# PalamaraLab/FastSMC

Measured on AMD Instinct MI355X. Metric: haplotype-pairs decoded/sec (whole node) + GB/s vs HBM roofline, 69-state HMM, higher is better.
Workload: dtype f32; 1 GPU; synthetic 1000 haplotypes x 50000 sites, K=69, all 499500 pairs per GPU, FastSMC-mode IBD + posterior-mean/MAP ages, no hashing; mode=ibd, resident_waves=2048, n_cu=256, chunk_sites=512, chunks_per_window=98, resident_chunks=24, beta_stride=2, kernel_member=69, record_gather=none, lib_hash=414cfd5268fcdcb0

## Files before the change

### fastsmc_amd/capi.py

```python
from __future__ import annotations

import ctypes as C
import operator
import os

import numpy as np

_HERE = os.path.dirname(os.path.abspath(__file__))
LIB_PATH = os.environ.get("FSMC_HIP_LIB") or os.path.join(_HERE, "libfastsmc_hip.so")

FSMC_WANT_MEAN = 1
FSMC_WANT_MAP = 2
FSMC_WANT_SUMS = 4
FSMC_WANT_MAJOR_MINOR_SUMS = 8

FSMC_EOVERFLOW = -6

SYMBOLS = [
    "fsmc_ctx_create", "fsmc_ctx_destroy", "fsmc_last_error", "fsmc_ctx_info", "fsmc_ctx_set_workspace_limit",
    "fsmc_ctx_expect_work",
    "fsmc_ctx_set_chunk_sites", "fsmc_ctx_set_beta_stride", "fsmc_ctx_last_beta_stride", "fsmc_ctx_last_plan",
    "fsmc_ctx_last_kernel", "fsmc_ctx_set_pairing", "fsmc_ctx_last_items", "fsmc_ctx_set_two_wave_windows", "fsmc_ctx_last_waves_per_window", "fsmc_ctx_last_segment_sums_in_lds", "fsmc_ctx_set_resident_chunks",
    "fsmc_ctx_last_resident_chunks", "fsmc_ctx_set_chunk_pool", "fsmc_ctx_last_chunk_pool",
    "fsmc_model_create", "fsmc_model_destroy", "fsmc_haps_upload", "fsmc_worklist_upload",
    "fsmc_decode_ibd_launch", "fsmc_decode_ibd_fetch", "fsmc_sync", "fsmc_last_kernel_ms", "fsmc_phase_cycles",
    "fsmc_decode_ibd",
    "fsmc_decode_posteriors", "fsmc_decode_per_pair", "fsmc_decode_sums", "fsmc_decode_sums_batches",
    "fsmc_decode_pair_posteriors", "fsmc_ctx_set_pair_posterior_slice", "fsmc_ctx_last_pair_posterior_slices",
    "fsmc_decode_pair_minima", "fsmc_ctx_set_pair_minima_slice", "fsmc_ctx_last_pair_minima_slices",
    "fsmc_decode_pair_bins", "fsmc_ctx_set_pair_bins_slice", "fsmc_ctx_last_pair_bins_slices",
    "fsmc_decode_pair_cdf", "fsmc_ctx_set_pair_cdf_slice", "fsmc_ctx_last_pair_cdf_slices",
    "fsmc_decode_pair_tail_summaries", "fsmc_ctx_set_pair_tail_slice", "fsmc_ctx_last_pair_tail_slices",
    "fsmc_decode_pair_loglik", "fsmc_ctx_set_pair_loglik_slice", "fsmc_ctx_last_pair_loglik_slices",
    "fsmc_decode_pair_viterbi", "fsmc_ctx_set_pair_viterbi_slice", "fsmc_ctx_last_pair_viterbi_slices",
    "fsmc_decode_pair_samples", "fsmc_ctx_set_pair_samples_slice", "fsmc_ctx_last_pair_samples_slices",
    "fsmc_identify", "fsmc_identify_ex", "fsmc_identify_fetch",
]

PAIR_DTYPE = np.dtype([("hap_a", "<u4"), ("hap_b", "<u4")])
GROUP_DTYPE = np.dtype([("first_pair", "<u4"), ("n_pairs", "<u4"), ("from", "<u4"), ("to", "<u4"),
                        ("scan_from", "<u4"), ("scan_to", "<u4")])
CANDIDATE_DTYPE = np.dtype([("hap_a", "<u4"), ("hap_b", "<u4"), ("from", "<u4"), ("to", "<u4"), ("flush_word", "<u4")])
IBD_DTYPE = np.dtype([("pair", "<u4"), ("start", "<i4"), ("end", "<i4"), ("prob", "<f4"), ("post_mean", "<f4"),
                      ("map", "<f4")])


def log_likelihood(mant, expo):
    with np.errstate(divide="ignore"):
        return np.log(np.asarray(mant, np.float64)) + np.asarray(expo, np.float64) * np.log(2.0)


class FsmcError(RuntimeError):
    def __init__(self, code: int, msg: str):
# ... 13 lines not shown

class _ModelDesc(C.Structure):
    _fields_ = [
        ("K", C.c_int32), ("S", C.c_int32),
        ("pi", C.c_void_p), ("col_ratios", C.c_void_p), ("exp_times", C.c_void_p),
        ("n_rows", C.c_int32),
        ("D", C.c_void_p), ("B", C.c_void_p), ("U", C.c_void_p), ("RR", C.c_void_p),
        ("step_row", C.c_void_p),
        ("e1", C.c_void_p), ("e0m1", C.c_void_p), ("e2m0", C.c_void_p),
        ("state_threshold", C.c_uint32), ("age_threshold", C.c_uint32), ("probability_threshold", C.c_float),
        ("sequence", C.c_int32),
        ("gap_row_f", C.c_void_p), ("site_row_f", C.c_void_p), ("gap_row_b", C.c_void_p), ("site_row_b", C.c_void_p),
        ("hom", C.c_void_p),
    ]


_lib = None


def load():
    global _lib
    if _lib is None:
        if not os.path.exists(LIB_PATH):
            raise FsmcError(-100, f"{LIB_PATH} is missing: build it with `python -c 'import __graft_entry__ as g; "
                                  "g.build()'` (there is no CPU fallback)")
        L = C.CDLL(LIB_PATH)
        vp, i32, u32, u64, sz = C.c_void_p, C.c_int32, C.c_uint32, C.c_uint64, C.c_size_t
        L.fsmc_ctx_create.argtypes = [C.c_int, vp, C.POINTER(vp)]
        L.fsmc_ctx_destroy.argtypes = [vp]
        L.fsmc_ctx_destroy.restype = None
        L.fsmc_last_error.argtypes = [vp]
        L.fsmc_last_error.restype = C.c_char_p
        L.fsmc_ctx_info.argtypes = [vp, C.POINTER(i32), C.POINTER(i32), C.POINTER(u64)]
        L.fsmc_ctx_set_workspace_limit.argtypes = [vp, u64]
        L.fsmc_ctx_expect_work.argtypes = [vp, C.c_double, C.c_int32]
        L.fsmc_ctx_set_chunk_sites.argtypes = [vp, u32]
        L.fsmc_ctx_set_beta_stride.argtypes = [vp, u32]
        L.fsmc_ctx_last_beta_stride.argtypes = [vp, C.POINTER(i32)]
        L.fsmc_ctx_last_plan.argtypes = [vp, C.POINTER(i32), C.POINTER(i32), C.POINTER(i32)]
        L.fsmc_ctx_last_kernel.argtypes = [vp, C.POINTER(i32)]
        L.fsmc_ctx_set_pairing.argtypes = [vp, u32]
        L.fsmc_ctx_set_two_wave_windows.argtypes = [vp, u32]
        L.fsmc_ctx_last_waves_per_window.argtypes = [vp, C.POINTER(i32)]
        L.fsmc_ctx_last_items.argtypes = [vp, C.POINTER(i32)]
        L.fsmc_ctx_last_segment_sums_in_lds.argtypes = [vp, C.POINTER(i32)]
        L.fsmc_ctx_set_chunk_pool.argtypes = [vp, i32, u32]
        L.fsmc_ctx_last_chunk_pool.argtypes = [vp, C.POINTER(u32), C.POINTER(u32), C.POINTER(u32), C.POINTER(u32)]
        L.fsmc_model_create.argtypes = [vp, C.POINTER(_ModelDesc), C.POINTER(vp)]
        L.fsmc_model_destroy.argtypes = [vp]
        L.fsmc_model_destroy.restype = None
        L.fsmc_haps_upload.argtypes = [vp, vp, u32, u32]
        L.fsmc_worklist_upload.argtypes = [vp, vp, sz, vp, sz]
        L.fsmc_decode_ibd_launch.argtypes = [vp, vp, u32]
        L.fsmc_decode_ibd_fetch.argtypes = [vp, vp, sz, C.POINTER(sz)]
        L.fsmc_sync.argtypes = [vp]
        L.fsmc_last_kernel_ms.argtypes = [vp, C.POINTER(C.c_float)]
        L.fsmc_phase_cycles.argtypes = [vp, vp, sz]
        L.fsmc_decode_ibd.argtypes = [vp, vp, vp, sz, vp, sz, u32, vp, sz, C.POINTER(sz)]
        L.fsmc_decode_posteriors.argtypes = [vp, vp, vp, sz]
        L.fsmc_decode_per_pair.argtypes = [vp, vp, vp, vp, vp]
        L.fsmc_decode_pair_posteriors.argtypes = [vp, vp, vp, vp, vp]
        L.fsmc_ctx_set_pair_posterior_slice.argtypes = [vp, u32]
        L.fsmc_ctx_last_pair_posterior_slices.argtypes = [vp, C.POINTER(i32)]
        L.fsmc_decode_pair_minima.argtypes = [vp, vp, vp, u64, vp, vp, vp, vp]
        L.fsmc_ctx_set_pair_minima_slice.argtypes = [vp, u32]
        L.fsmc_ctx_last_pair_minima_slices.argtypes = [vp, C.POINTER(i32)]
# ... 45 lines not shown
class Context:

    def __init__(self, device: int = 0, stream: int | None = None):
        self._L = load()
        h = C.c_void_p()
        rc = self._L.fsmc_ctx_create(device, C.c_void_p(stream) if stream else None, C.byref(h))
        if rc != 0:
            raise FsmcError(rc, (self._L.fsmc_last_error(None) or b"").decode())
        self._h = h
        self._models = []

    def _check(self, rc: int):
        if rc != 0:
            raise FsmcError(rc, (self._L.fsmc_last_error(self._h) or b"").decode())

    def close(self):
        if getattr(self, "_h", None):
            for m in list(self._models):
                m.close()
            self._L.fsmc_ctx_destroy(self._h)
            self._h = None

    def __del__(self):
        try:
            self.close()
        except Exception:
            pass

    def info(self) -> dict:
        cu, slots, hbm = C.c_int32(), C.c_int32(), C.c_uint64()
        self._check(self._L.fsmc_ctx_info(self._h, C.byref(cu), C.byref(slots), C.byref(hbm)))
        chunk, chunks = C.c_int32(), C.c_int32()
        self._check(self._L.fsmc_ctx_last_plan(self._h, C.byref(chunk), C.byref(chunks), None))
        return {"n_cu": cu.value, "n_slots": slots.value, "hbm_bytes": hbm.value, "chunk_sites": chunk.value,
                "max_chunks": chunks.value}

    def set_chunk_sites(self, sites: int):
        self._check(self._L.fsmc_ctx_set_chunk_sites(self._h, sites))

    def set_resident_chunks(self, chunks: int):
        self._check(self._L.fsmc_ctx_set_resident_chunks(self._h, chunks))

    def last_resident_chunks(self) -> int:
        v = C.c_int32(0)
        self._check(self._L.fsmc_ctx_last_resident_chunks(self._h, C.byref(v)))
        return v.value

    def set_chunk_pool(self, mode: int, phi_percent: int = 0):
        self._check(self._L.fsmc_ctx_set_chunk_pool(self._h, mode, phi_percent))

    def last_chunk_pool(self) -> dict:
        b, k, r, o = C.c_uint32(0), C.c_uint32(0), C.c_uint32(0), C.c_uint32(0)
        self._check(self._L.fsmc_ctx_last_chunk_pool(self._h, C.byref(b), C.byref(k), C.byref(r), C.byref(o)))
        return {"buffers": b.value, "kept": k.value, "rebuilt": r.value, "outstanding": o.value}

    def set_beta_stride(self, stride: int):
        self._check(self._L.fsmc_ctx_set_beta_stride(self._h, stride))

    def last_beta_stride(self) -> int:
        v = C.c_int32(0)
        self._check(self._L.fsmc_ctx_last_beta_stride(self._h, C.byref(v)))
        return v.value

    def last_kernel(self) -> int:
        v = C.c_int32(0)
        self._check(self._L.fsmc_ctx_last_kernel(self._h, C.byref(v)))
        return v.value

# ... 429 lines not shown
```

### fastsmc_amd/csrc/fsmc_capi.hip

```cpp
#include <hip/hip_runtime.h>

#include <algorithm>
#include <chrono>
#include <cmath>
#include <cstdio>
#include <cstdlib>
#include <cstring>
#include <new>
#include <string>
#include <type_traits>
#include <vector>

#include "fsmc_identify.h"
#include "fsmc_instances.h"
#include "fsmc_model_tables.h"
#include "fsmc_pair_bins.h"
#include "fsmc_pair_cdf.h"
#include "fsmc_pair_layout.h"
#include "fsmc_pair_tail.h"
#include "fsmc_pair_minima.h"
#include "fsmc_pair_posteriors.h"
#include "fsmc_plan.h"

namespace fsmc
{
hipError_t idSortCandidates(hipStream_t stream, const fsmc_candidate* in, fsmc_candidate* sorted, unsigned n,
                            unsigned nHaps, unsigned nWords);
hipError_t idSeedDepths(hipStream_t stream, const unsigned long long* words, unsigned nHaps, unsigned nWords,
                        unsigned maxSeeds, unsigned readAhead, unsigned char* depthOut,
                        unsigned hapStride);
}

using namespace fsmc;

namespace fsmc
{
__global__ void add_planes_in_order_kernel(const float* __restrict__ planes, float* __restrict__ acc, size_t n,
                                           int nPlanes, size_t planeStride)
{
  for (size_t i = (size_t)blockIdx.x * blockDim.x + threadIdx.x; i < n; i += (size_t)gridDim.x * blockDim.x) {
    float s = acc[i];
    for (int sl = 0; sl < nPlanes; ++sl) {
      s = s + planes[(size_t)sl * planeStride + i];
    }
    acc[i] = s;
  }
}
}

namespace
{
thread_local std::string g_createError;

struct DevBuf {
  void* p = nullptr;
  size_t bytes = 0;
};

constexpr int kChunkPoolDefault = -1;
constexpr uint32_t kChunkPoolPhiDefault = 200;

enum PairSlicing {
  kSlicePosteriors,
  kSliceMinima,
  kSliceBins,
  kSliceCdf,
  kSliceTail,
  kSliceLoglik,
  kSliceViterbi,
  kSliceSamples,
  kPairSlicings
};
}

struct fsmc_ctx {
  int device = 0;
  hipStream_t stream = nullptr;
  bool ownStream = false;
  int nCU = 0;
  uint64_t hbmBytes = 0;
  uint64_t wsLimit = 0;
  plan::Credit credit;
  std::string err;

  unsigned long long* dHaps = nullptr;
  uint32_t nHaps = 0, nSites = 0, W = 0;

  fsmc_pair* dPairs = nullptr;
  fsmc_group* dGroups = nullptr;
  size_t nPairs = 0, nGroups = 0;
  std::vector<fsmc_pair> hPairs;
  std::vector<fsmc_group> hGroups;

  unsigned* dCounters = nullptr;
  unsigned long long* dPhase = nullptr;
  DevBuf ws;
  DevBuf recs;
  size_t recCap = 0;
  DevBuf aux;
  DevBuf out;

  hipEvent_t ev0 = nullptr, ev1 = nullptr;
  bool timed = false;
  int lastSlots = 0;
  int lastChunk = 0, lastMaxChunks = 0, lastResident = 0;
  int residentChunks = -1;
  int chunkPool = kChunkPoolDefault;
  uint32_t chunkPoolPhi = kChunkPoolPhiDefault;
  DevBuf poolState;
  uint32_t lastPoolBuffers = 0;
  uint32_t chunkSites = 0;
  uint32_t betaStride = 0;
  int lastStride = 1;
  bool lastSpsLds = false;
  int lastMember = 0;
// ... 401 lines not shown
  d.maxSlots = envCount("FSMC_DIAG_MAX_SLOTS");
  d.wavesPerCU = envCount("FSMC_DIAG_WAVES_PER_CU");
  d.sumsSlots = envCount("FSMC_DIAG_SUMS_SLOTS");
  d.minimaRange = envCount("FSMC_DIAG_MINIMA_RANGE");
  if (const char* v = std::getenv("FSMC_DIAG_WS_FREE")) {
    d.wsFree = std::strtoull(v, nullptr, 10);
  }
  if (const char* v = std::getenv("FSMC_DIAG_WS_EARN_SCALE")) {
    d.earnScale = std::atof(v);
  }
  if (const char* v = std::getenv("FSMC_DIAG_TWO_WAVE_WINDOWS")) {
    d.twoWavesNever = std::strcmp(v, "never") == 0;
  }
  if (const char* v = std::getenv("FSMC_DIAG_W2_MEMBER")) {
    int nw = 0, kh = 0;
    if (std::sscanf(v, "%dx%d", &nw, &kh) == 2) {
      d.w2NW = nw;
      d.w2KH = kh;
    }
  }
  return d;
}

plan::Settings settingsOf(const fsmc_ctx* ctx)
{
  plan::Settings s;
  s.nCU = ctx->nCU;
  s.hbmBytes = ctx->hbmBytes;
  s.wsLimit = ctx->wsLimit;
  s.chunkSites = ctx->chunkSites;
  s.residentChunks = ctx->residentChunks;
  s.chunkPool = ctx->chunkPool;
  s.chunkPoolPhi = ctx->chunkPoolPhi;
  return s;
}

plan::MemInfo memInfo()
{
  size_t freeB = 0, totalB = 0;
  plan::MemInfo mem;
  mem.known = hipMemGetInfo(&freeB, &totalB) == hipSuccess;
  mem.freeBytes = (uint64_t)freeB;
  return mem;
}

hipError_t workgroupsPerCU(const KernelChoice& k, int most, int capDivisor, int& perCU)
{
  perCU = 0;
  const hipError_t e = hipOccupancyMaxActiveBlocksPerMultiprocessor(&perCU, k.fn, (int)k.threads, 0);
  if (e != hipSuccess) {
    (void)hipGetLastError();
    return e;
  }
  perCU = plan::capWorkgroups(perCU, most, capDivisor, readDiag());
  return hipSuccess;
}

static_assert(plan::kWave == kWave && plan::kFloat4Bytes == sizeof(float4), "fsmc_plan.h lays rows out for the kernels' wave");
static_assert(layout::kSpecBytes == sizeof(PairCdfSpec), "fsmc_pair_layout.h sizes pcSpec for the kernels' PairCdfSpec");

struct LaunchPlan : plan::LaunchPlan {
  KernelChoice k;
};

plan::KernelTraits traitsOf(const fsmc_model* m, int mode, const KernelChoice& k, int perCU)
{
  const bool w2 = waveGroups(mode, m);
  const bool any = anyStates(m);
  plan::KernelTraits t;
  t.member = k.member;
  t.stride = k.stride;
  t.rowFloat4 = w2 ? (size_t)m->KP / 4 : (size_t)((k.member > 0 ? k.member : m->K) + 3) / 4 + (any ? 1 : 0);
  t.sideRows = any ? (size_t)kAnyExtraRows + 2 : 4;
  t.chunkFloor = w2 ? 2048 : 512;
  t.resident = (mode == kModeIbd || mode == kModeSums) && !m->sequence && !any && (!w2 || w2ResidentBuilt(m->w2NW, false));
  t.pool = !w2 && k.poolFn != nullptr;
  t.perCU = perCU;
  return t;
}

plan::WsBudget workspaceBudget(const fsmc_ctx* ctx, const DevBuf& cur)
{
  return plan::workspaceBudget(settingsOf(ctx), ctx->credit, memInfo(), cur.bytes, readDiag());
}

void earnWorkspace(fsmc_ctx* ctx, const fsmc_model* m, int mode)
{
  plan::earnWorkspace(ctx->credit, ctx->hGroups, mode == kModeIbd, m->K, readDiag());
}

int planOneWave(const fsmc_ctx* ctx, const fsmc_model* m, int mode, const KernelChoice& k,
                const std::vector<fsmc_group>& list, bool paired, const plan::WsBudget& budget, unsigned share,
                LaunchPlan& plan, std::string& why)
{
  if (!k.fn) {
    why = "no kernel for this model";
    return FSMC_EUNSUPPORTED;
  }
  int perCU = 0;
  const hipError_t e = workgroupsPerCU(k, anyStates(m) ? 4 : 8, 1, perCU);
  if (e != hipSuccess) {
    why = std::string("occupancy query of the decode kernel: ") + hipGetErrorString(e);
    return FSMC_EHIP;
  }
  plan.k = k;
  return plan::planOneWave(settingsOf(ctx), traitsOf(m, mode, k, perCU), mode == kModeIbd, list, paired, budget, share,
                           readDiag(), plan, why);
}

int planViterbi(const fsmc_ctx* ctx, const fsmc_model* m, const KernelChoice& k, size_t nGroups, bool wantStates,
                const plan::WsBudget& budget, LaunchPlan& plan, std::string& why)
{
  int perCU = 0;
  const hipError_t e = workgroupsPerCU(k, 8, 1, perCU);
  if (e != hipSuccess) {
    why = std::string("occupancy query of the Viterbi kernel: ") + hipGetErrorString(e);
    return FSMC_EHIP;
  }
  plan.k = k;
  return plan::planViterbi(settingsOf(ctx), m->S, k.member, perCU, nGroups, wantStates, budget, plan, why);
}

int planSamples(const fsmc_ctx* ctx, const fsmc_model* m, const KernelChoice& k, size_t nGroups,
                const plan::WsBudget& budget, LaunchPlan& plan, std::string& why)
{
  int perCU = 0;
  const hipError_t e = workgroupsPerCU(k, 8, 1, perCU);
  if (e != hipSuccess) {
    why = std::string("occupancy query of the sampling kernel: ") + hipGetErrorString(e);
    return FSMC_EHIP;
  }
  plan.k = k;
  return plan::planSamples(settingsOf(ctx), m->S, k.member, perCU, nGroups, budget, plan, why);
}

bool twoWavesWanted(const fsmc_ctx* ctx, const KernelChoice& k2, size_t nItems)
{
  if (ctx->twoWaves == 1 || nItems == 0 || !k2.fn || readDiag().twoWavesNever) {
    return false;
  }
  int perCU = 0;
  return workgroupsPerCU(k2, 4, 2, perCU) == hipSuccess && plan::allResident(settingsOf(ctx), perCU, nItems);
}

bool planTwoWaves(const fsmc_ctx* ctx, const KernelChoice& k2, size_t nItems, const plan::WsBudget& budget, LaunchPlan& plan)
{
  plan.k = k2;
  return plan::planTwoWaves(ctx->hGroups, k2.member, nItems, budget, plan);
}

int holdWorkspace(fsmc_ctx* ctx, DevBuf& buf, size_t bytes)
{
  const char* most = std::getenv("FSMC_DIAG_WS_ALLOC_MAX");
  if (most && bytes > std::strtoull(most, nullptr, 10) && !(buf.p && buf.bytes >= bytes)) {
    if (buf.p) {
      (void)hipFree(buf.p);
    }
    buf = DevBuf();
    return fail(ctx, FSMC_ENOMEM, "workspace of " + std::to_string(bytes) + " bytes refused (FSMC_DIAG_WS_ALLOC_MAX)");
  }
  const size_t held = buf.bytes;
  const int rc = ensure(ctx, buf, bytes);
  if (rc != FSMC_OK) {
    (void)hipGetLastError();
  } else if (buf.bytes != held) {
    plan::payForWorkspace(settingsOf(ctx), ctx->credit, buf.bytes, readDiag());
  }
  return rc;
}

int planAndHold(fsmc_ctx* ctx, const fsmc_model* m, int mode, const KernelChoice& k, const std::vector<fsmc_group>& list,
                bool paired, unsigned share, DevBuf& buf, LaunchPlan& plan)
{
  std::string why;
  const int rc = planOneWave(ctx, m, mode, k, list, paired, workspaceBudget(ctx, buf), share, plan, why);
  if (rc != FSMC_OK) {
    return fail(ctx, rc, why);
  }
  if (plan.poolBuffers) {
    FSMC_TRY(ensure(ctx, ctx->poolState, (kPoolClaims + (size_t)plan.poolBuffers) * sizeof(unsigned)));
  }
  return holdWorkspace(ctx, buf, plan.bytes);
}

void recordLaunch(fsmc_ctx* ctx, const KernelChoice& k, const LaunchPlan& plan, int slotsBeside = 0)
{
  ctx->lastMember = k.member;
  ctx->lastStride = k.stride;
  ctx->lastChunk = plan.chunk;
  ctx->lastMaxChunks = plan.maxChunks;
  ctx->lastResident = plan.residentChunks;
  ctx->lastPoolBuffers = plan.poolBuffers;
  ctx->lastWavesPerWindow = plan.wavesPerWindow;
  ctx->lastSlots = plan.slots + slotsBeside;
}

int checkReady(fsmc_ctx* ctx, const fsmc_model* m)
{
  if (!ctx || !m) {
    return fail(ctx, FSMC_EINVAL, "null context or model");
  }
  if (m->ctx != ctx) {
    return fail(ctx, FSMC_EINVAL, "model belongs to another context");
  }
  if (!ctx->dHaps) {
    return fail(ctx, FSMC_ESTATE, "no haplotypes uploaded (fsmc_haps_upload)");
  }
  if (!ctx->dPairs || !ctx->dGroups || ctx->nGroups == 0) {
    return fail(ctx, FSMC_ESTATE, "no work list uploaded (fsmc_worklist_upload)");
  }
  if ((uint32_t)m->S != ctx->nSites) {
    return fail(ctx, FSMC_EINVAL, "model has " + std::to_string(m->S) + " sites but haplotypes have " +
                                      std::to_string(ctx->nSites));
  }
// ... 497 lines not shown
  if (e == hipSuccess) e = hipStreamCreateWithFlags(&ctx->side, hipStreamNonBlocking);
  if (e == hipSuccess) e = hipEventCreateWithFlags(&ctx->evFork, hipEventDisableTiming);
  if (e == hipSuccess) e = hipEventCreateWithFlags(&ctx->evJoin, hipEventDisableTiming);
  if (e == hipSuccess) e = hipMalloc((void**)&ctx->dCounters, 4 * sizeof(unsigned));
  if (e == hipSuccess) e = hipMalloc((void**)&ctx->dPhase, kPhaseSlots * sizeof(unsigned long long));
  if (e == hipSuccess) e = hipMemset(ctx->dPhase, 0, kPhaseSlots * sizeof(unsigned long long));
  if (e != hipSuccess) {
    std::string msg = std::string("context set-up failed: ") + hipGetErrorString(e);
    fsmc_ctx_destroy(ctx);
    return fail(nullptr, FSMC_EHIP, msg);
  }
  {
    int blocks = 0;
    const hipError_t pe = hipOccupancyMaxActiveBlocksPerMultiprocessor(
      &blocks, decode_kernel<128, kModeIbd, true, false, false>, kWave, 0);
    if (pe != hipSuccess) {
      (void)hipGetLastError();
      const std::vector<std::string> rts = mappedHipRuntimes();
      std::string msg = std::string("kernels of this library cannot be launched (") + hipGetErrorString(pe) + ")";
      int code = FSMC_EHIP;
      if (rts.size() > 1) {
        code = FSMC_ERUNTIME;
        msg += ": two HIP runtimes are loaded in this process (";
        for (size_t i = 0; i < rts.size(); ++i) {
          msg += (i ? ", " : "") + rts[i];
        }
        msg += "): load one libamdhip64 only -- e.g. import torch before this library so that both resolve to the "
               "copy torch bundles, or link both against the same ROCm";
      }
      fsmc_ctx_destroy(ctx);
      return fail(nullptr, code, msg);
    }
  }
  *out = ctx;
  return FSMC_OK;
}

void fsmc_ctx_destroy(fsmc_ctx* ctx)
{
  if (!ctx) {
    return;
  }
  (void)hipSetDevice(ctx->device);
  if (ctx->stream) {
    (void)hipStreamSynchronize(ctx->stream);
  }
  if (ctx->dHaps) (void)hipFree(ctx->dHaps);
  if (ctx->dPairs) (void)hipFree(ctx->dPairs);
  if (ctx->dGroups) (void)hipFree(ctx->dGroups);
  if (ctx->dItems) (void)hipFree(ctx->dItems);
  if (ctx->dRest) (void)hipFree(ctx->dRest);
  if (ctx->dCounters) (void)hipFree(ctx->dCounters);
  if (ctx->poolState.p) (void)hipFree(ctx->poolState.p);
  if (ctx->dPhase) (void)hipFree(ctx->dPhase);
  if (ctx->idStash.p) (void)hipFree(ctx->idStash.p);
  if (ctx->ws.p) (void)hipFree(ctx->ws.p);
  if (ctx->recs.p) (void)hipFree(ctx->recs.p);
  if (ctx->aux.p) (void)hipFree(ctx->aux.p);
  if (ctx->out.p) (void)hipFree(ctx->out.p);
  if (ctx->ev0) (void)hipEventDestroy(ctx->ev0);
  if (ctx->ev1) (void)hipEventDestroy(ctx->ev1);
  if (ctx->evFork) (void)hipEventDestroy(ctx->evFork);
  if (ctx->evJoin) (void)hipEventDestroy(ctx->evJoin);
  if (ctx->side) (void)hipStreamDestroy(ctx->side);
  if (ctx->wsSide.p) (void)hipFree(ctx->wsSide.p);
  if (ctx->copyStream) (void)hipStreamSynchronize(ctx->copyStream);
  if (ctx->ppStage.p) (void)hipFree(ctx->ppStage.p);
  if (ctx->ppRows.p) (void)hipFree(ctx->ppRows.p);
  if (ctx->pcSpec.p) (void)hipFree(ctx->pcSpec.p);
  if (ctx->ptAcc.p) (void)hipFree(ctx->ptAcc.p);
  if (ctx->ppAcc.p) (void)hipFree(ctx->ppAcc.p);
  if (ctx->pmAcc.p) (void)hipFree(ctx->pmAcc.p);
  if (ctx->pbAcc.p) (void)hipFree(ctx->pbAcc.p);
  if (ctx->plAcc.p) (void)hipFree(ctx->plAcc.p);
  if (ctx->pvAcc.p) (void)hipFree(ctx->pvAcc.p);
  for (int i = 0; i < 2; ++i) {
    if (ctx->ppPinned[i]) (void)hipHostFree(ctx->ppPinned[i]);
    if (ctx->evCopied[i]) (void)hipEventDestroy(ctx->evCopied[i]);
  }
  if (ctx->evRows) (void)hipEventDestroy(ctx->evRows);
  if (ctx->copyStream) (void)hipStreamDestroy(ctx->copyStream);
  if (ctx->ownStream && ctx->stream) (void)hipStreamDestroy(ctx->stream);
  delete ctx;
}

int fsmc_ctx_info(const fsmc_ctx* ctx, int32_t* n_cu, int32_t* n_slots, uint64_t* hbm_bytes)
{
  if (!ctx) {
    return FSMC_EINVAL;
  }
  if (n_cu) *n_cu = ctx->nCU;
  if (n_slots) *n_slots = ctx->lastSlots;
  if (hbm_bytes) *hbm_bytes = ctx->hbmBytes;
  return FSMC_OK;
}

int fsmc_ctx_set_workspace_limit(fsmc_ctx* ctx, uint64_t bytes)
{
  if (!ctx) {
    return FSMC_EINVAL;
  }
  ctx->wsLimit = bytes;
  return FSMC_OK;
}

int fsmc_ctx_expect_work(fsmc_ctx* ctx, double pair_sites, int32_t states)
{
  if (!ctx) {
    return fail(nullptr, FSMC_EINVAL, "null context");
  }
  if (!(pair_sites >= 0) || states < 1) {
    return fail(ctx, FSMC_EINVAL, "expected work: pair-sites >= 0 and states >= 1");
  }
  plan::expectWork(settingsOf(ctx), ctx->credit, pair_sites, states, readDiag());
  return FSMC_OK;
}

int fsmc_ctx_set_chunk_sites(fsmc_ctx* ctx, uint32_t sites)
{
  if (!ctx) {
    return FSMC_EINVAL;
  }
  ctx->chunkSites = sites;
  return FSMC_OK;
}

// ... 1537 lines not shown
```

### fastsmc_amd/csrc/fsmc_plan.h

```cpp
#pragma once

#include <algorithm>
#include <cmath>
#include <cstddef>
#include <cstdint>
#include <string>
#include <vector>

#include "../../include/fastsmc_hip.h"

namespace fsmc
{
namespace plan
{
constexpr int kWave = 64;
constexpr size_t kFloat4Bytes = 16;

struct Settings {
  int nCU = 0;
  uint64_t hbmBytes = 0;
  uint64_t wsLimit = 0;
  uint32_t chunkSites = 0;
  int residentChunks = -1;
  int chunkPool = -1;
  uint32_t chunkPoolPhi = 200;
};

struct MemInfo {
  bool known = false;
  uint64_t freeBytes = 0;
};

struct KernelTraits {
  int member = 0;
  int stride = 1;
  size_t rowFloat4 = 0;
  size_t sideRows = 4;
  size_t chunkFloor = 512;
  bool resident = false;
  bool pool = false;
  int perCU = 0;
};

struct LaunchPlan {
  int chunk = 0;
  int chunkRows = 0;
  int maxChunks = 0;
  int residentChunks = 0;
  size_t wsSlot = 0;
  int slots = 0;
  int wavesPerWindow = 1;
  size_t bytes = 0;
  size_t poolOff = 0;
  uint32_t poolBuffers = 0;
  int poolCap = 0;
};

constexpr double kAllocBytesPerSecond = 25e9;
constexpr double kEarnFraction = 0.06;
constexpr uint64_t kFreeWorkspace = 24ull << 30;

struct Diag {
  long maxSlots = 0;
  long wavesPerCU = 0;
  long sumsSlots = 0;
  uint64_t wsFree = kFreeWorkspace;
  double earnScale = 1.0;
  bool twoWavesNever = false;
  int w2NW = 0, w2KH = 0;
  long minimaRange = 0;
};

inline size_t lowered(size_t value, long n, int divisor = 1)
{
  const long v = n / divisor;
  return v >= 1 && (size_t)v < value ? (size_t)v : value;
}

inline int capWorkgroups(int counted, int most, int capDivisor, const Diag& diag)
{
  int perCU = std::min(counted, most);
  if (capDivisor > 0) {
    perCU = (int)lowered((size_t)std::max(perCU, 0), diag.wavesPerCU, capDivisor);
  }
  return perCU;
}

struct WsBudget {
  uint64_t hard, soft;
};

struct Credit {
  double earned = 0;
  double announced = 0;
  double announcedCredit = 0;
};

inline WsBudget workspaceBudget(const Settings& set, const Credit& credit, const MemInfo& mem, uint64_t curBytes,
                                const Diag& diag)
{
  const uint64_t reachable = mem.freeBytes + curBytes;
  const uint64_t margin = (uint64_t)(0.04 * (double)set.hbmBytes);
  if (set.wsLimit) {
    uint64_t lim = set.wsLimit;
    if (mem.known && reachable > margin && reachable - margin < lim && reachable - margin >= lim / 4) {
      lim = reachable - margin;
    }
    return {lim, lim};
  }
  const uint64_t floor40 = (uint64_t)(0.40 * (double)set.hbmBytes);
  uint64_t hard = floor40;
  if (mem.known) {
    const uint64_t want = (uint64_t)(0.80 * (double)set.hbmBytes);
    hard = std::max<uint64_t>(floor40, std::min<uint64_t>(want, reachable > margin ? reachable - margin : 0));
  }
  uint64_t earned = (uint64_t)std::min(std::max(credit.earned, 0.0), 1e15);
  if (earned < hard && earned < 2 * curBytes) {
    earned = 0;
  }
  const uint64_t freeBytes = diag.wsFree;
  const uint64_t soft = std::min<uint64_t>(hard, std::max<uint64_t>({curBytes, earned, freeBytes}));
  return {hard, soft};
}

inline void payForWorkspace(const Settings& set, Credit& credit, uint64_t allocatedBytes, const Diag& diag)
{
  if (set.wsLimit) {
    return;
  }
  const uint64_t freeBytes = diag.wsFree;
  if (allocatedBytes > freeBytes) {
    credit.earned = std::max(0.0, credit.earned - (double)(allocatedBytes - freeBytes));
  }
}

inline uint32_t windowEnd(const fsmc_group& g, bool ibd)
{
  return ibd ? g.scan_to : g.to;
}

inline double kernelSeconds(double pairSites, int states)
{
  return pairSites * (8.0 * states + 0.25) / (0.8 * 8e12);
}

inline void earnWorkspace(Credit& credit, const std::vector<fsmc_group>& groups, bool ibd, int states, const Diag& diag)
{
  double pairSites = 0;
  for (const fsmc_group& g : groups) {
    const uint32_t aEnd = windowEnd(g, ibd);
    pairSites += (double)g.n_pairs * (double)(aEnd > g.from ? aEnd - g.from : 0);
  }
  double seconds = kernelSeconds(pairSites, states);
  const double announced = std::min(credit.announced, seconds);
  if (credit.announced > 0) {
    credit.announcedCredit *= (credit.announced - announced) / credit.announced;
  }
  credit.announced -= announced;
  seconds -= announced;
  credit.earned += diag.earnScale * kEarnFraction * seconds * kAllocBytesPerSecond;
}

inline void expectWork(const Settings& set, Credit& credit, double pairSites, int states, const Diag& diag)
{
  if (pairSites == 0) {
    credit.earned = std::max(0.0, credit.earned - credit.announcedCredit);
    credit.announced = 0;
    credit.announcedCredit = 0;
    return;
  }
  const double seconds = kernelSeconds(pairSites, states);
  const double given = std::min(diag.earnScale * kEarnFraction * seconds * kAllocBytesPerSecond,
                                std::max(0.0, (double)set.hbmBytes - credit.announcedCredit));
  credit.announced += seconds;
  credit.announcedCredit += given;
  credit.earned += given;
}

inline int planOneWave(const Settings& set, const KernelTraits& k, bool ibd, const std::vector<fsmc_group>& list,
                       bool paired, const WsBudget& budget, unsigned share, const Diag& diag, LaunchPlan& plan,
                       std::string& why)
{
  const size_t slots =
      lowered(std::max<size_t>(1, std::min((size_t)set.nCU * std::max(k.perCU, 1), list.size())), diag.maxSlots);
  size_t L = 1;
  for (const fsmc_group& g : list) {
    const size_t aEnd = windowEnd(g, ibd);
    L = std::max<size_t>(L, aEnd - g.from);
  }
  const size_t K4 = k.rowFloat4;
  const size_t vecBytes = K4 * kWave * kFloat4Bytes;
  const uint64_t limit = budget.hard / share;
  const bool half = k.stride == 2;
  auto chunkRows = [&](size_t c) { return half ? (c + 1) / 2 : c; };
  const size_t rowsAvail = (size_t)(limit / (vecBytes * slots));
  const size_t rowsSoft = (size_t)(budget.soft / share / (vecBytes * slots));
  const size_t sideRows = k.sideRows;
  const size_t defaultChunk = std::max<size_t>((size_t)std::ceil(std::sqrt((double)L)), k.chunkFloor);
  size_t C, maxChunks;
  if (chunkRows(L) + sideRows + 1 <= rowsAvail && (chunkRows(L) + sideRows + 1 <= rowsSoft || L <= defaultChunk) &&
      !(set.chunkSites && set.chunkSites < L)) {
    C = L;
    maxChunks = 1;
  } else {
    C = set.chunkSites ? (size_t)set.chunkSites : defaultChunk;
// ... 326 lines not shown
```

### include/fastsmc_hip.h

```cpp
#ifndef FASTSMC_HIP_H
#define FASTSMC_HIP_H

#include <stddef.h>
#include <stdint.h>

#ifdef __cplusplus
extern "C" {
#endif

#define FSMC_OK 0
#define FSMC_EINVAL (-1)
#define FSMC_ENODEVICE (-2)
#define FSMC_EHIP (-3)
#define FSMC_ENOMEM (-4)
#define FSMC_ESTATE (-5)
#define FSMC_EOVERFLOW (-6)
#define FSMC_EUNSUPPORTED (-7)
#define FSMC_ERUNTIME (-8)

typedef struct fsmc_ctx fsmc_ctx;
typedef struct fsmc_model fsmc_model;

typedef struct {
  int32_t K;
// ... 21 lines not shown
  const float* hom;
} fsmc_model_desc;

typedef struct {
  uint32_t hap_a;
  uint32_t hap_b;
} fsmc_pair;

typedef struct {
  uint32_t first_pair;
  uint32_t n_pairs;
  uint32_t from, to;
  uint32_t scan_from, scan_to;
} fsmc_group;

typedef struct {
  uint32_t pair;
  int32_t start;
  int32_t end;
  float prob;
  float post_mean;
  float map;
} fsmc_ibd_record;

#define FSMC_WANT_MEAN 1u
#define FSMC_WANT_MAP 2u
#define FSMC_WANT_SUMS 4u
#define FSMC_WANT_MAJOR_MINOR_SUMS 8u

int fsmc_ctx_create(int device_id, void* stream, fsmc_ctx** out);
void fsmc_ctx_destroy(fsmc_ctx* ctx);
const char* fsmc_last_error(const fsmc_ctx* ctx);
int fsmc_ctx_info(const fsmc_ctx* ctx, int32_t* n_cu, int32_t* n_slots, uint64_t* hbm_bytes);
int fsmc_ctx_set_workspace_limit(fsmc_ctx* ctx, uint64_t bytes);
int fsmc_ctx_expect_work(fsmc_ctx* ctx, double pair_sites, int32_t states);
int fsmc_ctx_set_chunk_sites(fsmc_ctx* ctx, uint32_t sites);
int fsmc_ctx_set_beta_stride(fsmc_ctx* ctx, uint32_t stride);
int fsmc_ctx_last_beta_stride(const fsmc_ctx* ctx, int32_t* stride);
int fsmc_ctx_last_plan(const fsmc_ctx* ctx, int32_t* chunk_sites, int32_t* max_chunks, int32_t* n_slots);
int fsmc_ctx_set_resident_chunks(fsmc_ctx* ctx, int32_t chunks);
int fsmc_ctx_last_resident_chunks(const fsmc_ctx* ctx, int32_t* chunks);
int fsmc_ctx_set_chunk_pool(fsmc_ctx* ctx, int32_t mode, uint32_t phi_percent);
int fsmc_ctx_last_chunk_pool(fsmc_ctx* ctx, uint32_t* buffers, uint32_t* kept, uint32_t* rebuilt, uint32_t* outstanding);
int fsmc_ctx_set_pairing(fsmc_ctx* ctx, uint32_t mode);
int fsmc_ctx_last_items(const fsmc_ctx* ctx, int32_t* n_items);
int fsmc_ctx_set_two_wave_windows(fsmc_ctx* ctx, uint32_t mode);
int fsmc_ctx_last_waves_per_window(const fsmc_ctx* ctx, int32_t* waves);
int fsmc_ctx_last_segment_sums_in_lds(const fsmc_ctx* ctx, int32_t* in_lds);
int fsmc_ctx_set_pair_posterior_slice(fsmc_ctx* ctx, uint32_t groups);
int fsmc_ctx_last_pair_posterior_slices(const fsmc_ctx* ctx, int32_t* slices);
int fsmc_ctx_set_pair_minima_slice(fsmc_ctx* ctx, uint32_t groups);
int fsmc_ctx_last_pair_minima_slices(const fsmc_ctx* ctx, int32_t* slices);
int fsmc_ctx_set_pair_bins_slice(fsmc_ctx* ctx, uint32_t groups);
int fsmc_ctx_last_pair_bins_slices(const fsmc_ctx* ctx, int32_t* slices);
int fsmc_ctx_set_pair_cdf_slice(fsmc_ctx* ctx, uint32_t groups);
int fsmc_ctx_last_pair_cdf_slices(const fsmc_ctx* ctx, int32_t* slices);
int fsmc_ctx_set_pair_tail_slice(fsmc_ctx* ctx, uint32_t groups);
int fsmc_ctx_last_pair_tail_slices(const fsmc_ctx* ctx, int32_t* slices);
int fsmc_ctx_set_pair_loglik_slice(fsmc_ctx* ctx, uint32_t groups);
int fsmc_ctx_last_pair_loglik_slices(const fsmc_ctx* ctx, int32_t* slices);
int fsmc_ctx_set_pair_viterbi_slice(fsmc_ctx* ctx, uint32_t groups);
int fsmc_ctx_last_pair_viterbi_slices(const fsmc_ctx* ctx, int32_t* slices);
int fsmc_ctx_set_pair_samples_slice(fsmc_ctx* ctx, uint32_t groups);
int fsmc_ctx_last_pair_samples_slices(const fsmc_ctx* ctx, int32_t* slices);
int fsmc_ctx_last_kernel(const fsmc_ctx* ctx, int32_t* member);

// ... 83 lines not shown
```

Before: 283,200 pairs/s.

## Back decode workspace with growable virtual-memory mapped chunks instead of hipMalloc

```diff
diff --git a/fastsmc_amd/capi.py b/fastsmc_amd/capi.py
--- a/fastsmc_amd/capi.py
+++ b/fastsmc_amd/capi.py
@@ -17,8 +17,8 @@
 FSMC_EOVERFLOW = -6
 
 SYMBOLS = [
-    "fsmc_ctx_create", "fsmc_ctx_destroy", "fsmc_last_error", "fsmc_ctx_info", "fsmc_ctx_set_workspace_limit",
-    "fsmc_ctx_expect_work",
+    "fsmc_ctx_create", "fsmc_ctx_destroy", "fsmc_last_error", "fsmc_ctx_info", "fsmc_ctx_workspace_info",
+    "fsmc_ctx_set_workspace_limit", "fsmc_ctx_expect_work",
     "fsmc_ctx_set_chunk_sites", "fsmc_ctx_set_beta_stride", "fsmc_ctx_last_beta_stride", "fsmc_ctx_last_plan",
     "fsmc_ctx_last_kernel", "fsmc_ctx_set_pairing", "fsmc_ctx_last_items", "fsmc_ctx_set_two_wave_windows", "fsmc_ctx_last_waves_per_window", "fsmc_ctx_last_segment_sums_in_lds", "fsmc_ctx_set_resident_chunks",
     "fsmc_ctx_last_resident_chunks", "fsmc_ctx_set_chunk_pool", "fsmc_ctx_last_chunk_pool",
@@ -98,6 +98,7 @@
         L.fsmc_last_error.argtypes = [vp]
         L.fsmc_last_error.restype = C.c_char_p
         L.fsmc_ctx_info.argtypes = [vp, C.POINTER(i32), C.POINTER(i32), C.POINTER(u64)]
+        L.fsmc_ctx_workspace_info.argtypes = [vp, C.POINTER(i32), C.POINTER(i32), C.POINTER(u64), C.POINTER(u64)]
         L.fsmc_ctx_set_workspace_limit.argtypes = [vp, u64]
         L.fsmc_ctx_expect_work.argtypes = [vp, C.c_double, C.c_int32]
         L.fsmc_ctx_set_chunk_sites.argtypes = [vp, u32]
@@ -209,8 +210,13 @@
         self._check(self._L.fsmc_ctx_info(self._h, C.byref(cu), C.byref(slots), C.byref(hbm)))
         chunk, chunks = C.c_int32(), C.c_int32()
         self._check(self._L.fsmc_ctx_last_plan(self._h, C.byref(chunk), C.byref(chunks), None))
+        backing, handles, held, base = C.c_int32(), C.c_int32(), C.c_uint64(), C.c_uint64()
+        self._check(self._L.fsmc_ctx_workspace_info(self._h, C.byref(backing), C.byref(handles), C.byref(held),
+                                                    C.byref(base)))
         return {"n_cu": cu.value, "n_slots": slots.value, "hbm_bytes": hbm.value, "chunk_sites": chunk.value,
-                "max_chunks": chunks.value}
+                "max_chunks": chunks.value,
+                "ws_backing": "mapped" if backing.value == 1 else "malloc", "ws_handles": handles.value,
+                "ws_bytes": held.value, "ws_base": base.value}
 
     def set_chunk_sites(self, sites: int):
         self._check(self._L.fsmc_ctx_set_chunk_sites(self._h, sites))
diff --git a/fastsmc_amd/csrc/fsmc_capi.hip b/fastsmc_amd/csrc/fsmc_capi.hip
--- a/fastsmc_amd/csrc/fsmc_capi.hip
+++ b/fastsmc_amd/csrc/fsmc_capi.hip
@@ -11,6 +11,7 @@
 #include <type_traits>
 #include <vector>
 
+#include "fsmc_chunk_buf.h"
 #include "fsmc_identify.h"
 #include "fsmc_instances.h"
 #include "fsmc_model_tables.h"
@@ -55,7 +56,68 @@
 struct DevBuf {
   void* p = nullptr;
   size_t bytes = 0;
+  chunkbuf::ChunkBuf* chunks = nullptr;
 };
+
+class HipMapper : public chunkbuf::Mapper
+{
+public:
+  int device = 0;
+  bool reserve(size_t bytes, size_t alignment, void** base) override
+  {
+    return hipMemAddressReserve(base, bytes, alignment, nullptr, 0) == hipSuccess;
+  }
+  void unreserve(void* base, size_t bytes) override { (void)hipMemAddressFree(base, bytes); }
+  bool create(size_t bytes, uint64_t* handle) override
+  {
+    hipMemGenericAllocationHandle_t h = nullptr;
+    if (hipMemCreate(&h, bytes, &prop(), 0) != hipSuccess) {
+      return false;
+    }
+    *handle = (uint64_t)reinterpret_cast<uintptr_t>(h);
+    return true;
+  }
+  void release(uint64_t handle) override
+  {
+    (void)hipMemRelease(reinterpret_cast<hipMemGenericAllocationHandle_t>((uintptr_t)handle));
+  }
+  bool map(void* at, size_t bytes, uint64_t handle) override
+  {
+    return hipMemMap(at, bytes, 0, reinterpret_cast<hipMemGenericAllocationHandle_t>((uintptr_t)handle), 0) == hipSuccess;
+  }
+  bool allow(void* at, size_t bytes) override
+  {
+    hipMemAccessDesc desc = {};
+    desc.location = prop().location;
+    desc.flags = hipMemAccessFlagsProtReadWrite;
+    return hipMemSetAccess(at, bytes, &desc, 1) == hipSuccess;
+  }
+  void unmap(void* at, size_t bytes) override { (void)hipMemUnmap(at, bytes); }
+  const hipMemAllocationProp& prop()
+  {
+    prop_ = hipMemAllocationProp{};
+    prop_.type = hipMemAllocationTypePinned;
+    prop_.location.type = hipMemLocationTypeDevice;
+    prop_.location.id = device;
+    return prop_;
+  }
+  size_t granule()
+  {
+    size_t g = 0;
+    if (hipMemGetAllocationGranularity(&g, &prop(), hipMemAllocationGranularityRecommended) != hipSuccess) {
+      (void)hipGetLastError();
+      return 0;
+    }
+    return g;
+  }
+
+private:
+  hipMemAllocationProp prop_;
+};
+
+constexpr size_t kWsHandleBytes = (size_t)1 << 30;
+constexpr size_t kWsGranule = (size_t)2 << 20;
+constexpr bool kMapUnderLimit = true;
 
 constexpr int kChunkPoolDefault = -1;
 constexpr uint32_t kChunkPoolPhiDefault = 200;
@@ -81,6 +143,9 @@
   uint64_t hbmBytes = 0;
   uint64_t wsLimit = 0;
   plan::Credit credit;
+  HipMapper mapper;
+  bool wsMapped = false;
+  size_t mapGranule = 0, mapHandleBytes = 0;
   std::string err;
 
   unsigned long long* dHaps = nullptr;
@@ -548,6 +613,9 @@
   s.residentChunks = ctx->residentChunks;
   s.chunkPool = ctx->chunkPool;
   s.chunkPoolPhi = ctx->chunkPoolPhi;
+  if (ctx->wsMapped) {
+    s.allocBytesPerSecond = plan::kMappedBytesPerSecond;
+  }
   return s;
 }
 
@@ -602,7 +670,7 @@
 
 void earnWorkspace(fsmc_ctx* ctx, const fsmc_model* m, int mode)
 {
-  plan::earnWorkspace(ctx->credit, ctx->hGroups, mode == kModeIbd, m->K, readDiag());
+  plan::earnWorkspace(ctx->credit, ctx->hGroups, mode == kModeIbd, m->K, readDiag(), settingsOf(ctx).allocBytesPerSecond);
 }
 
 int planOneWave(const fsmc_ctx* ctx, const fsmc_model* m, int mode, const KernelChoice& k,
@@ -665,24 +733,97 @@
   return plan::planTwoWaves(ctx->hGroups, k2.member, nItems, budget, plan);
 }
 
+void initMappedWorkspace(fsmc_ctx* ctx)
+{
+  ctx->mapper.device = ctx->device;
+  ctx->wsMapped = false;
+  if (std::getenv("FSMC_DIAG_WS_NO_MAP")) {
+    return;
+  }
+  const size_t granule = ctx->mapper.granule();
+  if (granule == 0) {
+    return;
+  }
+  ctx->mapGranule = (kWsGranule + granule - 1) / granule * granule;
+  ctx->mapHandleBytes = kWsHandleBytes;
+  if (const char* v = std::getenv("FSMC_DIAG_WS_HANDLE_BYTES")) {
+    ctx->mapHandleBytes = std::max<size_t>(1, std::strtoull(v, nullptr, 10));
+  }
+  ctx->wsMapped = true;
+}
+
+chunkbuf::ChunkBuf* mappedChunks(fsmc_ctx* ctx, DevBuf& buf)
+{
+  if (buf.chunks || buf.p || !ctx->wsMapped || (!kMapUnderLimit && ctx->wsLimit)) {
+    return buf.chunks;
+  }
+  chunkbuf::ChunkBuf* chunks = new (std::nothrow) chunkbuf::ChunkBuf();
+  if (!chunks || !chunks->reserve(&ctx->mapper, (size_t)ctx->hbmBytes, ctx->mapHandleBytes, ctx->mapGranule)) {
+    (void)hipGetLastError();
+    delete chunks;
+    return nullptr;
+  }
+  buf.chunks = chunks;
+  return chunks;
+}
+
+void releaseWorkspace(DevBuf& buf)
+{
+  if (buf.chunks) {
+    delete buf.chunks;
+  } else if (buf.p) {
+    (void)hipFree(buf.p);
+  }
+  buf = DevBuf();
+}
+
 int holdWorkspace(fsmc_ctx* ctx, DevBuf& buf, size_t bytes)
 {
+  if (buf.p && buf.bytes >= bytes) {
+    return FSMC_OK;
+  }
   const char* most = std::getenv("FSMC_DIAG_WS_ALLOC_MAX");
-  if (most && bytes > std::strtoull(most, nullptr, 10) && !(buf.p && buf.bytes >= bytes)) {
-    if (buf.p) {
-      (void)hipFree(buf.p);
-    }
-    buf = DevBuf();
+  const bool refused = most && bytes > std::strtoull(most, nullptr, 10);
+  chunkbuf::ChunkBuf* chunks = mappedChunks(ctx, buf);
+  if (!chunks) {
+    if (refused) {
+      if (buf.p) {
+        (void)hipFree(buf.p);
+      }
+      buf = DevBuf();
+      return fail(ctx, FSMC_ENOMEM, "workspace of " + std::to_string(bytes) + " bytes refused (FSMC_DIAG_WS_ALLOC_MAX)");
+    }
+    const size_t held = buf.bytes;
+    const int rc = ensure(ctx, buf, bytes);
+    if (rc != FSMC_OK) {
+      (void)hipGetLastError();
+    } else if (buf.bytes != held) {
+      plan::payForWorkspace(settingsOf(ctx), ctx->credit, buf.bytes, readDiag());
+    }
+    return rc;
+  }
+  if (refused) {
     return fail(ctx, FSMC_ENOMEM, "workspace of " + std::to_string(bytes) + " bytes refused (FSMC_DIAG_WS_ALLOC_MAX)");
   }
   const size_t held = buf.bytes;
-  const int rc = ensure(ctx, buf, bytes);
-  if (rc != FSMC_OK) {
+  const bool timing = bytes - held >= (256u << 20) && std::getenv("FSMC_HOST_TIMING") != nullptr;
+  const auto t0 = std::chrono::steady_clock::now();
+  const size_t got = chunks->grow(bytes);
+  buf.p = got ? chunks->base() : nullptr;
+  buf.bytes = got;
+  if (timing) {
+    std::fprintf(stderr, "[fsmc] mapping %.2f GB behind %.2f GB took %.3f s\n", (double)(got - held) / 1e9,
+                 (double)held / 1e9, std::chrono::duration<double>(std::chrono::steady_clock::now() - t0).count());
+  }
+  if (got > held) {
+    plan::payForWorkspace(settingsOf(ctx), ctx->credit, got, readDiag(), held);
+  }
+  if (got < bytes) {
     (void)hipGetLastError();
-  } else if (buf.bytes != held) {
-    plan::payForWorkspace(settingsOf(ctx), ctx->credit, buf.bytes, readDiag());
-  }
-  return rc;
+    return fail(ctx, FSMC_ENOMEM, "workspace of " + std::to_string(bytes) + " bytes: " + std::to_string(got) +
+                                      " bytes could be mapped");
+  }
+  return FSMC_OK;
 }
 
 int planAndHold(fsmc_ctx* ctx, const fsmc_model* m, int mode, const KernelChoice& k, const std::vector<fsmc_group>& list,
@@ -696,6 +837,19 @@
   if (plan.poolBuffers) {
     FSMC_TRY(ensure(ctx, ctx->poolState, (kPoolClaims + (size_t)plan.poolBuffers) * sizeof(unsigned)));
   }
+  const int held = holdWorkspace(ctx, buf, plan.bytes);
+  if (held != FSMC_ENOMEM || !buf.chunks || buf.bytes == 0) {
+    return held;
+  }
+  const std::string refusal = ctx->err;
+  const plan::WsBudget within = {(uint64_t)buf.bytes * share, (uint64_t)buf.bytes * share};
+  if (planOneWave(ctx, m, mode, k, list, paired, within, share, plan, why) != FSMC_OK || plan.bytes > buf.bytes) {
+    return fail(ctx, FSMC_ENOMEM, refusal);
+  }
+  if (plan.poolBuffers) {
+    FSMC_TRY(ensure(ctx, ctx->poolState, (kPoolClaims + (size_t)plan.poolBuffers) * sizeof(unsigned)));
+  }
+  ctx->err.clear();
   return holdWorkspace(ctx, buf, plan.bytes);
 }
 
@@ -1259,6 +1413,7 @@
       return fail(nullptr, code, msg);
     }
   }
+  initMappedWorkspace(ctx);
   *out = ctx;
   return FSMC_OK;
 }
@@ -1281,7 +1436,7 @@
   if (ctx->poolState.p) (void)hipFree(ctx->poolState.p);
   if (ctx->dPhase) (void)hipFree(ctx->dPhase);
   if (ctx->idStash.p) (void)hipFree(ctx->idStash.p);
-  if (ctx->ws.p) (void)hipFree(ctx->ws.p);
+  releaseWorkspace(ctx->ws);
   if (ctx->recs.p) (void)hipFree(ctx->recs.p);
   if (ctx->aux.p) (void)hipFree(ctx->aux.p);
   if (ctx->out.p) (void)hipFree(ctx->out.p);
@@ -1290,7 +1445,7 @@
   if (ctx->evFork) (void)hipEventDestroy(ctx->evFork);
   if (ctx->evJoin) (void)hipEventDestroy(ctx->evJoin);
   if (ctx->side) (void)hipStreamDestroy(ctx->side);
-  if (ctx->wsSide.p) (void)hipFree(ctx->wsSide.p);
+  releaseWorkspace(ctx->wsSide);
   if (ctx->copyStream) (void)hipStreamSynchronize(ctx->copyStream);
   if (ctx->ppStage.p) (void)hipFree(ctx->ppStage.p);
   if (ctx->ppRows.p) (void)hipFree(ctx->ppRows.p);
@@ -1319,6 +1474,20 @@
   if (n_cu) *n_cu = ctx->nCU;
   if (n_slots) *n_slots = ctx->lastSlots;
   if (hbm_bytes) *hbm_bytes = ctx->hbmBytes;
+  return FSMC_OK;
+}
+
+int fsmc_ctx_workspace_info(const fsmc_ctx* ctx, int32_t* backing, int32_t* handles, uint64_t* bytes, uint64_t* base)
+{
+  if (!ctx) {
+    return FSMC_EINVAL;
+  }
+  const bool mapped = ctx->ws.chunks != nullptr || (!ctx->ws.p && ctx->wsMapped && (kMapUnderLimit || !ctx->wsLimit));
+  if (backing) *backing = mapped ? FSMC_WS_MAPPED : FSMC_WS_MALLOC;
+  if (handles) *handles = (int32_t)((ctx->ws.chunks ? ctx->ws.chunks->handles() : 0) +
+                                    (ctx->wsSide.chunks ? ctx->wsSide.chunks->handles() : 0));
+  if (bytes) *bytes = (uint64_t)ctx->ws.bytes + (uint64_t)ctx->wsSide.bytes;
+  if (base) *base = (uint64_t)reinterpret_cast<uintptr_t>(ctx->ws.p);
   return FSMC_OK;
 }
 
diff --git a/fastsmc_amd/csrc/fsmc_chunk_buf.h b/fastsmc_amd/csrc/fsmc_chunk_buf.h
--- /dev/null
+++ b/fastsmc_amd/csrc/fsmc_chunk_buf.h
@@ -0,0 +1,118 @@
+#pragma once
+
+#include <algorithm>
+#include <cstddef>
+#include <cstdint>
+#include <vector>
+
+namespace fsmc
+{
+namespace chunkbuf
+{
+class Mapper
+{
+public:
+  virtual ~Mapper() = default;
+  virtual bool reserve(size_t bytes, size_t alignment, void** base) = 0;
+  virtual void unreserve(void* base, size_t bytes) = 0;
+  virtual bool create(size_t bytes, uint64_t* handle) = 0;
+  virtual void release(uint64_t handle) = 0;
+  virtual bool map(void* at, size_t bytes, uint64_t handle) = 0;
+  virtual bool allow(void* at, size_t bytes) = 0;
+  virtual void unmap(void* at, size_t bytes) = 0;
+};
+
+class ChunkBuf
+{
+public:
+  ChunkBuf() = default;
+  ChunkBuf(const ChunkBuf&) = delete;
+  ChunkBuf& operator=(const ChunkBuf&) = delete;
+  ~ChunkBuf() { destroy(); }
+
+  bool reserve(Mapper* mapper, size_t rangeBytes, size_t handleBytes, size_t granule)
+  {
+    destroy();
+    if (!mapper || granule == 0 || rangeBytes == 0) {
+      return false;
+    }
+    granule_ = granule;
+    handleBytes_ = (std::max<size_t>(handleBytes, 1) + granule - 1) / granule * granule;
+    range_ = (rangeBytes + handleBytes_ - 1) / handleBytes_ * handleBytes_;
+    if (range_ < rangeBytes || !mapper->reserve(range_, granule_, &base_) || !base_) {
+      base_ = nullptr;
+      range_ = 0;
+      return false;
+    }
+    mapper_ = mapper;
+    return true;
+  }
+
+  size_t grow(size_t bytes)
+  {
+    if (!mapper_ || bytes > range_) {
+      return mapped_;
+    }
+    while (mapped_ < bytes && mapOne(handleBytes_)) {
+    }
+    return mapped_;
+  }
+
+  void destroy()
+  {
+    if (mapper_) {
+      while (!handles_.empty()) {
+        const Handle h = handles_.back();
+        handles_.pop_back();
+        mapped_ -= h.bytes;
+        mapper_->unmap(static_cast<char*>(base_) + mapped_, h.bytes);
+        mapper_->release(h.handle);
+      }
+      mapper_->unreserve(base_, range_);
+    }
+    mapper_ = nullptr;
+    base_ = nullptr;
+    range_ = mapped_ = 0;
+    handles_.clear();
+  }
+
+  bool reserved() const { return mapper_ != nullptr; }
+  void* base() const { return base_; }
+  size_t range() const { return range_; }
+  size_t mapped() const { return mapped_; }
+  size_t handles() const { return handles_.size(); }
+  size_t handleBytes() const { return handleBytes_; }
+
+private:
+  bool mapOne(size_t need)
+  {
+    char* const at = static_cast<char*>(base_) + mapped_;
+    uint64_t handle = 0;
+    if (!mapper_->create(need, &handle)) {
+      return false;
+    }
+    if (!mapper_->map(at, need, handle)) {
+      mapper_->release(handle);
+      return false;
+    }
+    if (!mapper_->allow(at, need)) {
+      mapper_->unmap(at, need);
+      mapper_->release(handle);
+      return false;
+    }
+    handles_.push_back({handle, need});
+    mapped_ += need;
+    return true;
+  }
+
+  struct Handle {
+    uint64_t handle;
+    size_t bytes;
+  };
+  Mapper* mapper_ = nullptr;
+  void* base_ = nullptr;
+  size_t granule_ = 0, handleBytes_ = 0, range_ = 0, mapped_ = 0;
+  std::vector<Handle> handles_;
+};
+}
+}
diff --git a/fastsmc_amd/csrc/fsmc_plan.h b/fastsmc_amd/csrc/fsmc_plan.h
--- a/fastsmc_amd/csrc/fsmc_plan.h
+++ b/fastsmc_amd/csrc/fsmc_plan.h
@@ -15,6 +15,9 @@
 {
 constexpr int kWave = 64;
 constexpr size_t kFloat4Bytes = 16;
+
+constexpr double kAllocBytesPerSecond = 25e9;
+constexpr double kMappedBytesPerSecond = kAllocBytesPerSecond;
 
 struct Settings {
   int nCU = 0;
@@ -24,6 +27,7 @@
   int residentChunks = -1;
   int chunkPool = -1;
   uint32_t chunkPoolPhi = 200;
+  double allocBytesPerSecond = kAllocBytesPerSecond;
 };
 
 struct MemInfo {
@@ -56,7 +60,6 @@
   int poolCap = 0;
 };
 
-constexpr double kAllocBytesPerSecond = 25e9;
 constexpr double kEarnFraction = 0.06;
 constexpr uint64_t kFreeWorkspace = 24ull << 30;
 
@@ -96,6 +99,15 @@
   double announcedCredit = 0;
 };
 
+inline uint64_t freeAllowance(const Settings& set, const Diag& diag)
+{
+  if (set.allocBytesPerSecond == kAllocBytesPerSecond) {
+    return diag.wsFree;
+  }
+  const double scaled = (double)diag.wsFree * (set.allocBytesPerSecond / kAllocBytesPerSecond);
+  return (uint64_t)std::min(std::max(scaled, 0.0), 1e18);
+}
+
 inline WsBudget workspaceBudget(const Settings& set, const Credit& credit, const MemInfo& mem, uint64_t curBytes,
                                 const Diag& diag)
 {
@@ -118,19 +130,20 @@
   if (earned < hard && earned < 2 * curBytes) {
     earned = 0;
   }
-  const uint64_t freeBytes = diag.wsFree;
+  const uint64_t freeBytes = freeAllowance(set, diag);
   const uint64_t soft = std::min<uint64_t>(hard, std::max<uint64_t>({curBytes, earned, freeBytes}));
   return {hard, soft};
 }
 
-inline void payForWorkspace(const Settings& set, Credit& credit, uint64_t allocatedBytes, const Diag& diag)
+inline void payForWorkspace(const Settings& set, Credit& credit, uint64_t allocatedBytes, const Diag& diag,
+                            uint64_t heldBytes = 0)
 {
   if (set.wsLimit) {
     return;
   }
-  const uint64_t freeBytes = diag.wsFree;
-  if (allocatedBytes > freeBytes) {
-    credit.earned = std::max(0.0, credit.earned - (double)(allocatedBytes - freeBytes));
+  const uint64_t paidFor = std::max<uint64_t>(freeAllowance(set, diag), heldBytes);
+  if (allocatedBytes > paidFor) {
+    credit.earned = std::max(0.0, credit.earned - (double)(allocatedBytes - paidFor));
   }
 }
 
@@ -144,7 +157,8 @@
   return pairSites * (8.0 * states + 0.25) / (0.8 * 8e12);
 }
 
-inline void earnWorkspace(Credit& credit, const std::vector<fsmc_group>& groups, bool ibd, int states, const Diag& diag)
+inline void earnWorkspace(Credit& credit, const std::vector<fsmc_group>& groups, bool ibd, int states, const Diag& diag,
+                          double allocBytesPerSecond = kAllocBytesPerSecond)
 {
   double pairSites = 0;
   for (const fsmc_group& g : groups) {
@@ -158,7 +172,7 @@
   }
   credit.announced -= announced;
   seconds -= announced;
-  credit.earned += diag.earnScale * kEarnFraction * seconds * kAllocBytesPerSecond;
+  credit.earned += diag.earnScale * kEarnFraction * seconds * allocBytesPerSecond;
 }
 
 inline void expectWork(const Settings& set, Credit& credit, double pairSites, int states, const Diag& diag)
@@ -170,7 +184,7 @@
     return;
   }
   const double seconds = kernelSeconds(pairSites, states);
-  const double given = std::min(diag.earnScale * kEarnFraction * seconds * kAllocBytesPerSecond,
+  const double given = std::min(diag.earnScale * kEarnFraction * seconds * set.allocBytesPerSecond,
                                 std::max(0.0, (double)set.hbmBytes - credit.announcedCredit));
   credit.announced += seconds;
   credit.announcedCredit += given;
diff --git a/include/fastsmc_hip.h b/include/fastsmc_hip.h
--- a/include/fastsmc_hip.h
+++ b/include/fastsmc_hip.h
@@ -77,6 +77,9 @@
 void fsmc_ctx_destroy(fsmc_ctx* ctx);
 const char* fsmc_last_error(const fsmc_ctx* ctx);
 int fsmc_ctx_info(const fsmc_ctx* ctx, int32_t* n_cu, int32_t* n_slots, uint64_t* hbm_bytes);
+#define FSMC_WS_MALLOC 0
+#define FSMC_WS_MAPPED 1
+int fsmc_ctx_workspace_info(const fsmc_ctx* ctx, int32_t* backing, int32_t* handles, uint64_t* bytes, uint64_t* base);
 int fsmc_ctx_set_workspace_limit(fsmc_ctx* ctx, uint64_t bytes);
 int fsmc_ctx_expect_work(fsmc_ctx* ctx, double pair_sites, int32_t states);
 int fsmc_ctx_set_chunk_sites(fsmc_ctx* ctx, uint32_t sites);
```

Result: no change. 284,500 pairs/s, median of 6 (+0.4%).
